# alonbebchuk/GNN-Pretraining

Hardware: AMD Instinct MI355X
Metric: pretrain graphs/sec (s4 multi-task) (higher is better)
Workload: dtype fp32; 1 GPU; s4 (NFM+LP+NC+GC+GP) pre-training step, 4 domains x 8 synthetic ENZYMES-shaped graphs per rank (input dims 7/4/37/21, hidden 256, 5 GIN layers), PCGrad + clip + AdamW; global_batch_graphs=32, parallelism=dp1, setup_steps=30, full=False, index_rng=reference, index_draws=native (csrc_host/hostdraw.cpp), cross_stream_sync=gates, ranks=1, devices_visible=1

## Files before the change

gnn_pretraining_amd/csrc/optim.hip:

```cpp
#include "gnnmp_internal.h"

namespace {

constexpr int MAXT = 8;
constexpr int CH = 32;
constexpr int GCH = 32;
constexpr int TB = 256;

struct MtArgs {
    const float* tg;
    int64_t stride;
    int T, K;
    int k0, k1;
    const int64_t* off;
    const int* len;
    const unsigned char* has;
    double* gram;
    double* gram_part;
    float* weights;
    int* flags;
    float* steps;
    int* metrics;
    int* block_metrics;
    int order[MAXT];
    int n_order;
    int last_task;
    int extra_task;
    float* final_grad;
    float* partial;
    float* normsq;
    float* params;
    float* exp_avg;
    float* exp_avg_sq;
    const float* lr;
    const float* wd;
    float beta1, beta2, eps, max_norm;
    const int* abort;
};

constexpr int MINP4 = 1024;
__device__ __forceinline__ int chunk_per4(int len4, int nch) { return max((len4 + nch - 1) / nch, MINP4); }
__device__ __forceinline__ int chunk_count(int len, int nch) {
    const int len4 = (len + 3) / 4;
    return len4 > 0 ? (len4 + chunk_per4(len4, nch) - 1) / chunk_per4(len4, nch) : 1;
}
__device__ __forceinline__ bool locate_chunk(const MtArgs& a, int k0, int k1, int nch, int b, int* k_out, int* j_out) {
    __shared__ int s_kj[2];
    if (threadIdx.x < 64) {
        const int lane = threadIdx.x;
        if (lane == 0) s_kj[0] = -1;
        int base = 0;
        for (int t0 = k0; t0 < k1; t0 += 64) {
            const int k = t0 + lane;
            const int cnt = k < k1 ? chunk_count(a.len[k], nch) : 0;
            int incl = cnt;
#pragma unroll
            for (int o = 1; o < 64; o <<= 1) {
                const int v = __shfl_up(incl, o, 64);
                if (lane >= o) incl += v;
            }
            const int excl = base + incl - cnt;
            if (cnt > 0 && b >= excl && b < excl + cnt) {
                s_kj[0] = k;
                s_kj[1] = b - excl;
            }
            base += __shfl(incl, 63, 64);
            if (base > b) break;
        }
    }
    __syncthreads();
    *k_out = s_kj[0];
    *j_out = s_kj[1];
    return s_kj[0] >= 0;
}

template <int NT>
__global__ __launch_bounds__(TB) void gram_kernel(const MtArgs a) {
    int k, j;
    if (!locate_chunk(a, a.k0, a.k1, GCH, blockIdx.x, &k, &j)) return;
    const int len = a.len[k], per = 4 * chunk_per4((len + 3) / 4, GCH);
    bool has[NT];
    int nh = 0;
#pragma unroll
    for (int t = 0; t < NT; ++t) {
        has[t] = t < a.T && a.has[k * MAXT + t];
        nh += has[t];
    }
    if (nh < 2) return;
    const int lo = j * per, hi = min(lo + per, (len + 3) / 4 * 4);
    double* out = a.gram_part + ((int64_t)k * GCH + j) * (MAXT * MAXT);
    constexpr int NP = NT * (NT + 1) / 2, NW = TB / 64, IT = 4;
    float acc[NP];
#pragma unroll
    for (int p = 0; p < NP; ++p) acc[p] = 0.f;
    const int64_t off = a.off[k];
    for (int i0 = lo + 4 * threadIdx.x; i0 < hi; i0 += IT * 4 * TB) {
        float4 g[IT][NT];
#pragma unroll
        for (int u = 0; u < IT; ++u) {
            const int i = i0 + u * 4 * TB;
#pragma unroll
            for (int t = 0; t < NT; ++t)
                g[u][t] = (has[t] && i < hi) ? *reinterpret_cast<const float4*>(a.tg + (int64_t)t * a.stride + off + i) : make_float4(0.f, 0.f, 0.f, 0.f);
        }
#pragma unroll
        for (int u = 0; u < IT; ++u) {
            int p = 0;
#pragma unroll
            for (int x = 0; x < NT; ++x)
#pragma unroll
                for (int y = x; y < NT; ++y, ++p) {
                    acc[p] += g[u][x].x * g[u][y].x;
                    acc[p] += g[u][x].y * g[u][y].y;
                    acc[p] += g[u][x].z * g[u][y].z;
                    acc[p] += g[u][x].w * g[u][y].w;
                }
        }
    }
    __shared__ double sh[NW][NP];
    const int lane = threadIdx.x % 64, wv = threadIdx.x / 64;
#pragma unroll
    for (int p = 0; p < NP; ++p) {
        float v = acc[p];
#pragma unroll
        for (int o = 32; o > 0; o >>= 1) v += __shfl_xor(v, o, 64);
        if (lane == 0) sh[wv][p] = (double)v;
    }
    __syncthreads();
    if (threadIdx.x < NP) {
        int x = 0, rem = threadIdx.x;
        while (rem >= NT - x) { rem -= NT - x; ++x; }
        const int y = x + rem;
        if (a.has[k * MAXT + x] && a.has[k * MAXT + y]) {
            double v = sh[0][threadIdx.x];
#pragma unroll
            for (int w = 1; w < NW; ++w) v += sh[w][threadIdx.x];
            out[x * MAXT + y] = v;
        }
    }
}

__global__ __launch_bounds__(64) void gram_finish_kernel(MtArgs a) {
    const int k = a.k0 + blockIdx.x, x = threadIdx.x / MAXT, y = threadIdx.x % MAXT;
    if (x >= a.T || y >= a.T || x > y) return;
    if (!a.has[k * MAXT + x] || !a.has[k * MAXT + y]) return;
    double s = 0.0;
    const int cnt = chunk_count(a.len[k], GCH);
    double v[GCH];
#pragma unroll
    for (int j = 0; j < GCH; ++j) v[j] = j < cnt ? a.gram_part[((int64_t)k * GCH + j) * (MAXT * MAXT) + x * MAXT + y] : 0.0;
#pragma unroll
    for (int j = 0; j < GCH; ++j) s += v[j];
    a.gram[((int64_t)k * MAXT + x) * MAXT + y] = s;
    a.gram[((int64_t)k * MAXT + y) * MAXT + x] = s;
}

__global__ __launch_bounds__(64) void solve_kernel(const MtArgs a) {
    __shared__ int s_conf[64], s_proj[64];
    int conf = 0, proj = 0;
    const int k = a.k0 + blockIdx.x * 64 + threadIdx.x;
    if (k < a.k1) {
        const unsigned char* has = a.has + k * MAXT;
        const double* G = a.gram + (int64_t)k * MAXT * MAXT;
        int flag = 0;
        float wout[MAXT];
#pragma unroll
        for (int i = 0; i < MAXT; ++i) wout[i] = 0.f;
        bool hp[MAXT];
        int nh = 0;
#pragma unroll
        for (int i = 0; i < MAXT; ++i) {
            hp[i] = i < a.n_order && has[a.order[i]];
            nh += hp[i];
        }
        if (nh > 1 || hp[0]) {
            double Gp[MAXT][MAXT];
#pragma unroll
            for (int i = 0; i < MAXT; ++i)
#pragma unroll
                for (int j = 0; j < MAXT; ++j) Gp[i][j] = (hp[i] && hp[j]) ? G[a.order[i] * MAXT + a.order[j]] : 0.0;
            double alpha[MAXT][MAXT];
#pragma unroll
            for (int i = 0; i < MAXT; ++i)
#pragma unroll
                for (int j = 0; j < MAXT; ++j) alpha[i][j] = i == j ? 1.0 : 0.0;
#pragma unroll
            for (int i = 1; i < MAXT; ++i) {
                if (!hp[i]) continue;
#pragma unroll
                for (int j = 0; j < i; ++j) {
                    if (!hp[j]) continue;
                    double ni = 0.0, dot = 0.0;
#pragma unroll
                    for (int p = 0; p <= i; ++p) {
                        double row = 0.0;
#pragma unroll
                        for (int q = 0; q <= i; ++q) row += alpha[i][q] * Gp[p][q];
                        ni += alpha[i][p] * row;
                        dot += alpha[i][p] * Gp[p][j];
                    }
                    const double nj = Gp[j][j];
                    if (ni <= 0.0 || nj <= 0.0) continue;
                    ++proj;
                    if (dot < 0.0) {
                        ++conf;
                        alpha[i][j] -= dot / nj;
                    }
                }
            }
#pragma unroll
            for (int i = 0; i < MAXT; ++i)
                if (hp[i]) {
#pragma unroll
                    for (int b = 0; b < MAXT; ++b) wout[b] += (float)(alpha[i][b] / nh);
                }
            flag = hp[0] ? 1 : 0;
        }
        float* w = a.weights + k * MAXT;
        for (int t = 0; t < MAXT; ++t) w[t] = 0.f;
        if (flag) {
#pragma unroll
            for (int i = 0; i < MAXT; ++i)
                if (i < a.n_order) w[a.order[i]] = wout[i];
        } else if (a.last_task >= 0 && has[a.last_task]) {
            w[a.last_task] = 1.f;
            flag = 1;
        }
        if (a.extra_task >= 0 && has[a.extra_task]) {
            w[a.extra_task] += 1.f;
            flag = 1;
        }
        a.flags[k] = flag;
        if (a.steps && !(a.abort && *a.abort)) a.steps[k] += (float)flag;
    }
    s_conf[threadIdx.x] = conf;
    s_proj[threadIdx.x] = proj;
    __syncthreads();
    for (int d = 32; d > 0; d >>= 1) {
        if (threadIdx.x < d) {
            s_conf[threadIdx.x] += s_conf[threadIdx.x + d];
            s_proj[threadIdx.x] += s_proj[threadIdx.x + d];
        }
        __syncthreads();
    }
    if (threadIdx.x == 0) {
        a.block_metrics[2 * (a.k0 + blockIdx.x)] = s_conf[0];
        a.block_metrics[2 * (a.k0 + blockIdx.x) + 1] = s_proj[0];
    }
    if (blockIdx.x == 0)
        for (int i = (int)gridDim.x + threadIdx.x; i < a.k1 - a.k0; i += 64) {
            a.block_metrics[2 * (a.k0 + i)] = 0;
            a.block_metrics[2 * (a.k0 + i) + 1] = 0;
        }
}

__global__ __launch_bounds__(TB) void combine_kernel(MtArgs a) {
    __shared__ float sh[TB / 64];
    int k, j;
    if (!locate_chunk(a, a.k0, a.k1, CH, blockIdx.x, &k, &j)) return;
    float ss = 0.f;
    if (a.flags[k]) {
        float w[MAXT];
        for (int t = 0; t < MAXT; ++t) w[t] = a.weights[k * MAXT + t];
        const int len4 = (a.len[k] + 3) / 4, per = chunk_per4(len4, CH);
        const int lo = j * per, hi = min(lo + per, len4);
        const int64_t off = a.off[k];
        for (int i = lo + threadIdx.x; i < hi; i += TB) {
            float4 g = make_float4(0.f, 0.f, 0.f, 0.f);
            for (int t = 0; t < a.T; ++t)
                if (w[t] != 0.f) {
                    const float4 v = *reinterpret_cast<const float4*>(a.tg + (int64_t)t * a.stride + off + 4 * (int64_t)i);
                    g = make_float4(fmaf(w[t], v.x, g.x), fmaf(w[t], v.y, g.y), fmaf(w[t], v.z, g.z), fmaf(w[t], v.w, g.w));
                }
            *reinterpret_cast<float4*>(a.final_grad + off + 4 * (int64_t)i) = g;
            ss = fmaf(g.x, g.x, ss); ss = fmaf(g.y, g.y, ss); ss = fmaf(g.z, g.z, ss); ss = fmaf(g.w, g.w, ss);
        }
    }
#pragma unroll
    for (int o = 32; o > 0; o >>= 1) ss += __shfl_xor(ss, o, 64);
    if (threadIdx.x % 64 == 0) sh[threadIdx.x / 64] = ss;
    __syncthreads();
    if (threadIdx.x == 0) {
        float s = sh[0];
        for (int w = 1; w < TB / 64; ++w) s += sh[w];
        a.partial[k * CH + j] = s;
    }
}

__global__ __launch_bounds__(TB) void foreign_kernel(MtArgs a) {
    __shared__ float sh[TB / 64];
    int k, j;
    if (!locate_chunk(a, a.k0, a.k1, CH, blockIdx.x, &k, &j)) return;
    const unsigned char* has = a.has + k * MAXT;
    int flag = a.n_order > 0 && has[a.order[0]] ? 1 : 0;
    if (!flag && a.last_task >= 0 && has[a.last_task]) flag = 1;
    if (a.extra_task >= 0 && has[a.extra_task]) flag = 1;
    if (j == 0 && threadIdx.x == 0) {
        a.flags[k] = flag;
        if (a.steps && !(a.abort && *a.abort)) a.steps[k] += (float)flag;
        a.block_metrics[2 * k] = 0;
        a.block_metrics[2 * k + 1] = 0;
    }
    float ss = 0.f;
    if (flag) {
        const int len4 = (a.len[k] + 3) / 4, per = chunk_per4(len4, CH);
        const int lo = j * per, hi = min(lo + per, len4);
        const int64_t off = a.off[k];
        for (int i = lo + threadIdx.x; i < hi; i += TB) {
            const float4 g = *reinterpret_cast<const float4*>(a.final_grad + off + 4 * (int64_t)i);
            ss = fmaf(g.x, g.x, ss); ss = fmaf(g.y, g.y, ss); ss = fmaf(g.z, g.z, ss); ss = fmaf(g.w, g.w, ss);
        }
    }
#pragma unroll
    for (int o = 32; o > 0; o >>= 1) ss += __shfl_xor(ss, o, 64);
    if (threadIdx.x % 64 == 0) sh[threadIdx.x / 64] = ss;
    __syncthreads();
    if (threadIdx.x == 0) {
        float s2 = sh[0];
        for (int w = 1; w < TB / 64; ++w) s2 += sh[w];
        a.partial[k * CH + j] = s2;
    }
}

__global__ __launch_bounds__(TB) void norm_kernel(MtArgs a) {
    __shared__ double sh[TB];
    __shared__ int shc[TB], shp[TB];
    double s = 0.0;
    for (int k = threadIdx.x; k < a.K; k += TB) {
        const int cnt = chunk_count(a.len[k], CH);
        const float4* row = reinterpret_cast<const float4*>(a.partial + (int64_t)k * CH);
        float4 v[CH / 4];
#pragma unroll
        for (int q = 0; q < CH / 4; ++q) v[q] = 4 * q < cnt ? row[q] : make_float4(0.f, 0.f, 0.f, 0.f);
#pragma unroll
        for (int q = 0; q < CH / 4; ++q) {
            if (4 * q + 0 < cnt) s += (double)v[q].x;
            if (4 * q + 1 < cnt) s += (double)v[q].y;
            if (4 * q + 2 < cnt) s += (double)v[q].z;
            if (4 * q + 3 < cnt) s += (double)v[q].w;
        }
    }
    int c = 0, pr = 0;
    for (int b = threadIdx.x; b < a.K; b += TB) {
        c += a.block_metrics[2 * b];
        pr += a.block_metrics[2 * b + 1];
    }
    sh[threadIdx.x] = s;
    shc[threadIdx.x] = c;
    shp[threadIdx.x] = pr;
    __syncthreads();
    for (int d = TB / 2; d > 0; d >>= 1) {
        if (threadIdx.x < d) {
            sh[threadIdx.x] += sh[threadIdx.x + d];
            shc[threadIdx.x] += shc[threadIdx.x + d];
            shp[threadIdx.x] += shp[threadIdx.x + d];
        }
        __syncthreads();
    }
    if (threadIdx.x == 0) {
        a.normsq[0] = (float)sh[0];
        a.metrics[0] = shc[0];
        a.metrics[1] = shp[0];
    }
}

__global__ __launch_bounds__(TB) void adamw_kernel(MtArgs a) {
    int k, j;
    if (!locate_chunk(a, 0, a.K, CH, blockIdx.x, &k, &j)) return;
    if (!a.flags[k]) return;
    if (a.abort && *a.abort) return;
    float coef = 1.f;
    if (a.max_norm > 0.f) coef = fminf(1.f, a.max_norm / (sqrtf(a.normsq[0]) + 1e-6f));
    const float lr = a.lr[k], wd = a.wd[k], step = a.steps[k];
    const float bc1 = 1.f - powf(a.beta1, step), bc2 = 1.f - powf(a.beta2, step);
    const float step_size = lr / bc1, bc2s = sqrtf(bc2);
    const int len4 = (a.len[k] + 3) / 4, per = chunk_per4(len4, CH);
    const int lo = j * per, hi = min(lo + per, len4);
    const int64_t off = a.off[k];
    auto one = [&](float g, float p, float m0, float v0, float* mo, float* vo) -> float {
        g *= coef;
        p *= (1.f - lr * wd);
        const float m = m0 + (g - m0) * (1.f - a.beta1);
        const float v = v0 * a.beta2 + g * g * (1.f - a.beta2);
        *mo = m;
        *vo = v;
        return p - step_size * (m / (sqrtf(v) / bc2s + a.eps));
    };
    for (int i = lo + threadIdx.x; i < hi; i += TB) {
        const int64_t o = off + 4 * (int64_t)i;
        const float4 g = *reinterpret_cast<const float4*>(a.final_grad + o), p = *reinterpret_cast<const float4*>(a.params + o);
        const float4 m0 = *reinterpret_cast<const float4*>(a.exp_avg + o), v0 = *reinterpret_cast<const float4*>(a.exp_avg_sq + o);
        float4 m, v, q;
        q.x = one(g.x, p.x, m0.x, v0.x, &m.x, &v.x);
        q.y = one(g.y, p.y, m0.y, v0.y, &m.y, &v.y);
        q.z = one(g.z, p.z, m0.z, v0.z, &m.z, &v.z);
        q.w = one(g.w, p.w, m0.w, v0.w, &m.w, &v.w);
        *reinterpret_cast<float4*>(a.exp_avg + o) = m;
        *reinterpret_cast<float4*>(a.exp_avg_sq + o) = v;
        *reinterpret_cast<float4*>(a.params + o) = q;
    }
}

}

extern "C" size_t gmp_mt_workspace_bytes(int num_tensors) {
    const size_t K = num_tensors > 0 ? num_tensors : 0;
    return K * MAXT * MAXT * sizeof(double) * (1 + GCH) + K * MAXT * sizeof(float) + K * sizeof(int) + K * CH * sizeof(float) +
           (K + 2) * 2 * sizeof(int) + 1024;
}

extern "C" int gmp_mt_pcgrad_clip_adamw_ex(const float* task_grads, int64_t task_stride, int num_tasks, int num_tensors,
                                           const int64_t* tensor_off, const int32_t* tensor_len, const uint8_t* has,
                                           const int32_t* order_host, int n_order, int last_task, int extra_task,
                                           float* params, float* exp_avg, float* exp_avg_sq, float* steps,
                                           const float* lr, const float* wd, float beta1, float beta2, float eps,
                                           float max_norm, float* final_grad, float* normsq_out, int32_t* metrics_out,
                                           int32_t* flags_out, void* ws, size_t ws_bytes, int apply_update,
                                           int k_begin, int k_end, int phases, const int32_t* abort_flag, gmp_stream_t stream) {
    if (k_begin < 0 || k_end > num_tensors || k_begin > k_end || !(phases & 7))
        return gmp::fail(GMP_ERR_ARG, "mt_pcgrad: tensors [%d, %d) of %d, phases %d", k_begin, k_end, num_tensors, phases);
    if (num_tasks < 1 || num_tasks > MAXT || num_tensors < 1 || n_order < 1 || n_order > num_tasks)
        return gmp::fail(GMP_ERR_ARG, "mt_pcgrad: tasks=%d tensors=%d n_order=%d", num_tasks, num_tensors, n_order);
    if (!task_grads || !tensor_off || !tensor_len || !has || !order_host || !final_grad || !normsq_out || !metrics_out || !flags_out || !ws)
        return gmp::fail(GMP_ERR_ARG, "mt_pcgrad: null pointer");
    if (apply_update && (!params || !exp_avg || !exp_avg_sq || !steps || !lr || !wd)) return gmp::fail(GMP_ERR_ARG, "mt_pcgrad: optimizer state");
    if (ws_bytes < gmp_mt_workspace_bytes(num_tensors)) return gmp::fail(GMP_ERR_WORKSPACE, "mt_pcgrad: workspace");
    if (last_task >= num_tasks || extra_task >= num_tasks) return gmp::fail(GMP_ERR_ARG, "mt_pcgrad: task index");
    MtArgs a{};
    a.tg = task_grads; a.stride = task_stride; a.T = num_tasks; a.K = num_tensors; a.off = tensor_off; a.len = tensor_len;
    a.k0 = k_begin; a.k1 = k_end;
    a.has = has;
    char* w = (char*)ws;
    a.gram = (double*)w; w += (size_t)num_tensors * MAXT * MAXT * sizeof(double);
    a.gram_part = (double*)w; w += (size_t)num_tensors * GCH * MAXT * MAXT * sizeof(double);
    a.weights = (float*)w; w += (size_t)num_tensors * MAXT * sizeof(float);
    a.partial = (float*)w; w += (size_t)num_tensors * CH * sizeof(float);
    a.block_metrics = (int*)w;
    a.flags = flags_out; a.steps = steps; a.metrics = metrics_out;
    for (int i = 0; i < n_order; ++i) {
        if (order_host[i] < 0 || order_host[i] >= num_tasks) return gmp::fail(GMP_ERR_ARG, "mt_pcgrad: order[%d]=%d", i, order_host[i]);
        a.order[i] = order_host[i];
    }
    a.n_order = n_order; a.last_task = last_task; a.extra_task = extra_task;
    a.final_grad = final_grad; a.normsq = normsq_out; a.params = params; a.exp_avg = exp_avg; a.exp_avg_sq = exp_avg_sq;
    a.lr = lr; a.wd = wd; a.beta1 = beta1; a.beta2 = beta2; a.eps = eps; a.max_norm = max_norm;
    a.abort = abort_flag;
    hipStream_t st = (hipStream_t)stream;
    const int nk = k_end - k_begin;
    auto nblk = [&](int n) { return (unsigned)(task_stride / (4 * MINP4) + 2 * (int64_t)n + 1); };
    if ((phases & 1) && nk > 0) {
        if (n_order > 1) {
            switch (num_tasks) {
                case 2: hipLaunchKernelGGL(gram_kernel<2>, dim3(nblk(nk)), dim3(TB), 0, st, a); break;
                case 3: hipLaunchKernelGGL(gram_kernel<3>, dim3(nblk(nk)), dim3(TB), 0, st, a); break;
                case 4: hipLaunchKernelGGL(gram_kernel<4>, dim3(nblk(nk)), dim3(TB), 0, st, a); break;
                case 5: hipLaunchKernelGGL(gram_kernel<5>, dim3(nblk(nk)), dim3(TB), 0, st, a); break;
                case 6: hipLaunchKernelGGL(gram_kernel<6>, dim3(nblk(nk)), dim3(TB), 0, st, a); break;
                default: hipLaunchKernelGGL(gram_kernel<MAXT>, dim3(nblk(nk)), dim3(TB), 0, st, a); break;
            }
            hipLaunchKernelGGL(gram_finish_kernel, dim3(nk), dim3(64), 0, st, a);
        }
        hipLaunchKernelGGL(solve_kernel, dim3((nk + 63) / 64), dim3(64), 0, st, a);
        hipLaunchKernelGGL(combine_kernel, dim3(nblk(nk)), dim3(TB), 0, st, a);
    }
    if ((phases & 4) && nk > 0) hipLaunchKernelGGL(foreign_kernel, dim3(nblk(nk)), dim3(TB), 0, st, a);
    if (phases & 2) {
        hipLaunchKernelGGL(norm_kernel, dim3(1), dim3(TB), 0, st, a);
        if (apply_update) hipLaunchKernelGGL(adamw_kernel, dim3(nblk(num_tensors)), dim3(TB), 0, st, a);
    }
    return gmp::check_launch("mt_pcgrad_clip_adamw kernels");
}

extern "C" int gmp_mt_pcgrad_clip_adamw(const float* task_grads, int64_t task_stride, int num_tasks, int num_tensors,
                                        const int64_t* tensor_off, const int32_t* tensor_len, const uint8_t* has,
                                        const int32_t* order_host, int n_order, int last_task, int extra_task,
                                        float* params, float* exp_avg, float* exp_avg_sq, float* steps,
                                        const float* lr, const float* wd, float beta1, float beta2, float eps,
                                        float max_norm, float* final_grad, float* normsq_out, int32_t* metrics_out,
                                        int32_t* flags_out, void* ws, size_t ws_bytes, int apply_update,
                                        gmp_stream_t stream) {
    return gmp_mt_pcgrad_clip_adamw_ex(task_grads, task_stride, num_tasks, num_tensors, tensor_off, tensor_len, has, order_host, n_order,
                                       last_task, extra_task, params, exp_avg, exp_avg_sq, steps, lr, wd, beta1, beta2, eps, max_norm,
                                       final_grad, normsq_out, metrics_out, flags_out, ws, ws_bytes, apply_update, 0, num_tensors, 3, nullptr, stream);
}
```

gnn_pretraining_amd/engine.py:

```python
from __future__ import annotations

import ctypes as C
import os
import random
from typing import Dict, List, Optional, Sequence, Tuple

import numpy as np
import torch
from torch import Tensor

from . import _lib as L
from .constants import DOMAIN_DIMENSIONS, GRAPH_PROPERTY_DIM
from .graph import Batch
from .models.gnn import DROPOUT_RATE, GNN_HIDDEN_DIM, GNN_NUM_LAYERS
from .models.pretrain_model import PretrainableGNN, draw_mask_indices
from .pretrain.augmentations import _augment_one
from .pretrain.control import DEFAULT_LR, DEFAULT_WEIGHT_DECAY, TASK_SPECIFIC_LR
from .pretrain.tasks import sample_negative_edges

H = GNN_HIDDEN_DIM
NT, NN, TN = 0, 1, 2
MAXT = 8
SEG_CSR_MAX_ROWS, SEG_CSR_MAX_EDGES = 8192, 24576

# ... 278 lines not shown
        return bool(self.use_gates and self.native and os.environ.get("GMP_UPLOAD_ON_AUX", "1") != "0")

    @property
    def parts_beside_backward(self) -> bool:
        return bool(self._parts_ok and self.native)

    def _flatten_parameters(self) -> None:
        m, dev = self.model, self.device
        named = dict(m.named_parameters())
        enc = [m.input_encoders[d] for d in self.domains]
        order: List[Tuple[str, Tensor]] = []
        for d, e in zip(self.domains, enc):
            order.append((f"input_encoders.{d}.linear.weight", e.linear.weight))
        for key in ("linear.bias", "batch_norm.weight", "batch_norm.bias"):
            for d in self.domains:
                order.append((f"input_encoders.{d}.{key}", named[f"input_encoders.{d}.{key}"]))
        seen = {n for n, _ in order}
        for n, p in named.items():
            if n not in seen:
                order.append((n, p))
        al4 = lambda v: (v + 3) // 4 * 4
        self.off: Dict[str, int] = {}
        o = 0
        for n, p in order:
            self.off[n] = o
            o += al4(p.numel())
        self.P = o
        self.P_shared = min(self.off[n] for n, _ in order if n.startswith("heads.")) if any(n.startswith("heads.") for n, _ in order) else o
        self.flat = torch.zeros(self.P, device=dev)
        for n, p in order:
            o = self.off[n]
            self.flat[o:o + p.numel()].copy_(p.data.reshape(-1))
            p.data = self.flat[o:o + p.numel()].view_as(p)
        self.names = [n for n, _ in order]
        self.numel = {n: p.numel() for n, p in order}
        self.enc_rm = torch.zeros(self.D, H, device=dev)
        self.enc_rv = torch.ones(self.D, H, device=dev)
        for i, e in enumerate(enc):
            self.enc_rm[i].copy_(e.batch_norm.running_mean)
            self.enc_rv[i].copy_(e.batch_norm.running_var)
            e.batch_norm.running_mean.data = self.enc_rm[i]
            e.batch_norm.running_var.data = self.enc_rv[i]
        self.exp_avg = torch.zeros(self.P, device=dev)
        self.exp_avg_sq = torch.zeros(self.P, device=dev)

    def _build_tables(self) -> None:
        dev, T = self.device, self.T
        K = len(self.names)
        self.K = K
        self.t_off = torch.tensor([self.off[n] for n in self.names], dtype=torch.int64, device=dev)
        self.t_len = torch.tensor([self.numel[n] for n in self.names], dtype=torch.int32, device=dev)
        has = np.zeros((K, MAXT), dtype=np.uint8)
        lr = np.zeros(K, dtype=np.float32)
        for k, n in enumerate(self.names):
            lr[k] = DEFAULT_LR
            if n.startswith("input_encoders."):
                for t, task in enumerate(self.tasks):
                    has[k, t] = task != "node_feat_mask"
            elif n == "mask_token":
                for t, task in enumerate(self.tasks):
                    has[k, t] = task == "node_feat_mask"
            elif n.startswith("gnn_backbone."):
                has[k, :T] = 1
            elif n.startswith("heads."):
                for t, task in enumerate(self.tasks):
                    if f"heads.{task}" in n:
                        has[k, t] = 1
                        lr[k] = TASK_SPECIFIC_LR[task]
        self.has_static = has
        self.has = torch.from_numpy(has.copy()).to(dev)
        self.lr = torch.from_numpy(lr).to(dev)
        self.wd = torch.full((K,), DEFAULT_WEIGHT_DECAY, dtype=torch.float32, device=dev)
        self.steps = torch.zeros(K, dtype=torch.float32, device=dev)
        self.name_index = {n: k for k, n in enumerate(self.names)}

    def _alloc(self) -> None:
        dev, R = self.device, self.max_rows
        f = lambda *shape: torch.empty(*shape, device=dev)
        self.task_grads = torch.zeros(self.T, self.P, device=dev)
        self.final_grad = torch.zeros(self.P, device=dev)
        self.normsq = torch.zeros(1, device=dev)
        self.metrics = torch.zeros(2, dtype=torch.int32, device=dev)
        self.flags = torch.zeros(self.K, dtype=torch.int32, device=dev)
        self.mt_ws = torch.empty(self.lib.gmp_mt_workspace_bytes(self.K), dtype=torch.uint8, device=dev)
        Lr = GNN_NUM_LAYERS
        self.z0 = f(R, H)
        self.h = [f(R, H) for _ in range(Lr + 1)]
        self.a = [f(R, H) for _ in range(Lr)]
        self.z1 = [f(R, 2 * H) for _ in range(Lr)]
        self.r1 = [f(R, 2 * H) for _ in range(Lr)]
        self.z2 = [f(R, H) for _ in range(Lr)]
        self.S_MAX = 64
        self.stat = {k: f(Lr, self.S_MAX, c) for k, c in (("m1", 2 * H), ("s1", 2 * H), ("m2", H), ("s2", H))}
        self.enc_mean, self.enc_rstd = f(self.S_MAX, H), f(self.S_MAX, H)
        self.gA, self.gB = f(R, H), f(R, H)
        self.ga = f(R, H)
        self.gW = f(R, 2 * H)
        self.gW2 = f(R, 2 * H)
        self.gB2, self.gW3 = f(R, H), f(R, 2 * H)
        self.gu_l, self.gz1_l = [f(R, H) for _ in range(Lr)], [f(R, 2 * H) for _ in range(Lr)]
        self.rowdot = f(Lr * R)
        self.gemm_ws = torch.empty(48 << 20, dtype=torch.uint8, device=dev)
        from . import streams as ST
        self.aux_stream, *extra = ST.concurrent_streams(dev, 3)
        self.sync_flags = torch.zeros(64, dtype=torch.int32, device=dev)
        self._epoch = 0
        self.use_gates = bool(ST.last_report.get("calibrated") and ST.last_report.get("own_queue") == 3
                              and os.environ.get("GMP_STEP_GATES", "1") != "0")
        self._parts_ok = (self.use_gates and os.environ.get("GMP_DP_OVERLAP", "1") != "0" and os.environ.get("GMP_OPT_OVERLAP", "0") == "1")
        self.comm_stream = extra[1]
        bins = [[0.0, extra[0]], [0.0, extra[1]], [0.0, self.aux_stream], [0.0, None]]
        self.task_streams = [None] * self.T
        for ti in sorted(range(self.T), key=lambda i: -HEAD_CHAIN_US.get(self.tasks[i], 100.0)):
            b = min(bins, key=lambda x: x[0])
            b[0] += HEAD_CHAIN_US.get(self.tasks[ti], 100.0)
            self.task_streams[ti] = b[1]
        self.task_gemm_ws = [torch.empty(24 << 20, dtype=torch.uint8, device=dev) for _ in range(self.T)]
        self.task_loss_ws = [torch.empty(self.lib.gmp_loss_workspace_bytes(R * H), dtype=torch.uint8, device=dev) for _ in range(self.T)]
        self._cur_gemm_ws = self.gemm_ws
        self.bn_ws = torch.empty(12 * self.lib.gmp_bn_workspace_bytes(R, 2 * H, self.S_MAX, R), dtype=torch.uint8, device=dev)
        self.csr_ws = torch.empty(self.lib.gmp_csr_build_workspace_bytes(R, self.max_edges), dtype=torch.uint8, device=dev)
        i32 = lambda n: torch.empty(n, dtype=torch.int32, device=dev)
        self.csr = [i32(R + 1), i32(self.max_edges), i32(self.max_edges), i32(R + 1), i32(self.max_edges), i32(self.max_edges)]
        self.csr_status = i32(1)
        self.lp_csr_status = i32(1)
        self.lp_csr_ws = torch.empty(self.lib.gmp_csr_build_workspace_bytes(R, self.max_edges), dtype=torch.uint8, device=dev)
        self.lp_csr = [i32(R + 1), i32(self.max_edges), i32(self.max_edges), i32(R + 1), i32(self.max_edges), i32(self.max_edges)]
        self.loss_sums = torch.zeros(MAXT, device=dev)
        self.loss_ws = torch.empty(self.lib.gmp_loss_workspace_bytes(R * H), dtype=torch.uint8, device=dev)
        self.KMAX = self.max_edges
        self.hd = {k: f(n, c) for k, (n, c) in {
            "nfm_in": (R, H), "nfm_y1": (R, H), "nfm_d1": (R, H), "nfm_y2": (R, H), "nfm_tgt": (R, H), "nfm_g": (R, H), "nfm_g1": (R, H), "nfm_gin": (R, H),
            "lp_feat": (self.KMAX, 3 * H), "lp_y1": (self.KMAX, H), "lp_d1": (self.KMAX, H), "lp_gy1": (self.KMAX, H),
            "lp_gfeat": (self.KMAX, 3 * H), "lp_ghs": (self.KMAX, H), "lp_ghd": (self.KMAX, H),
            "nc_in": (2 * R, H), "nc_y1": (2 * R, H), "nc_d1": (2 * R, H), "nc_z": (2 * R, 128), "nc_gz": (2 * R, 128), "nc_g1": (2 * R, H), "nc_gin": (2 * R, H),
            "gc_mean": (1024, H), "gc_max": (1024, H), "gc_in": (1024, 2 * H), "gc_y1": (1024, H), "gc_d1": (1024, H), "gc_z": (1024, 128),
            "gc_gz": (1024, 128), "gc_g1": (1024, H), "gc_gin": (1024, 2 * H), "gc_gmean": (1024, H), "gc_gmax": (1024, H),
            "da_in": (1024, H), "da_y1": (1024, DA_HIDDEN), "da_d1": (1024, DA_HIDDEN), "da_logits": (1024, 8), "da_glogits": (1024, 8),
            "da_g1": (1024, DA_HIDDEN), "da_gin": (1024, H),
            "gp_in": (1024, H), "gp_y1": (1024, 2 * H), "gp_d1": (1024, 2 * H), "gp_y2": (1024, 16), "gp_g2": (1024, 16), "gp_g1": (1024, 2 * H), "gp_gin": (1024, H),
        }.items()}
        self.lp_y2, self.lp_p, self.lp_gp, self.lp_gy2 = f(2 * self.KMAX), f(2 * self.KMAX), f(self.KMAX), f(2 * self.KMAX)
        self.gp_y2 = f(1024, GRAPH_PROPERTY_DIM)
        self.gp_g2 = f(1024, GRAPH_PROPERTY_DIM)
        self.ntx_ws = [torch.empty(self.lib.gmp_nt_xent_grouped_workspace_bytes(self.D, 512, 128), dtype=torch.uint8, device=dev) for _ in range(2 * self.D)]
        self.i32_cap, self.i64_cap = 4 * R + 8 * self.S_MAX + 65536 + 2 * self.max_edges, 4 * self.max_edges + 8 * R
        self.STAGES = 4
        self.stage = [{"pin32": torch.empty(self.i32_cap, dtype=torch.int32).pin_memory(),
                       "pin64": torch.empty(self.i64_cap, dtype=torch.int64).pin_memory(),
                       "pinf": torch.empty(64 + self.KMAX, dtype=torch.float32).pin_memory(),
                       "event": None} for _ in range(self.STAGES)]
        self._up_sets = [(torch.empty(self.i32_cap, dtype=torch.int32, device=dev), torch.empty(self.i64_cap, dtype=torch.int64, device=dev),
                          torch.zeros(64, device=dev), f(self.KMAX)) for _ in range(2)]
        self.dev32, self.dev64, self.scal, self.lp_lab = self._up_sets[0]

    def draw(self, inp: StepInputs, gen: torch.Generator) -> Dict[str, object]:
        if self.rng_mode == "vectorized":
            return self._draw_vectorized(inp, gen)
        if self.rng_mode == "device":
            return self.collect_draws(inp, self.enqueue_draws(inp))
        art: Dict[str, object] = {}
        host = {d: inp.host[d] for d in self.domains}
        H = hostdraw()
        if H is not None and hasattr(H, "draw_step"):
            if self._neg_native is None:
                self._neg_native = H.PyRandom()
                self._neg_native.setstate(torch.tensor(self.neg_rng.getstate()[1], dtype=torch.long))
# ... 1501 lines not shown
```

gnn_pretraining_amd/finetune/engine.py:

```python
from __future__ import annotations

import ctypes as C
import os as _os_mod
from typing import Dict, List, NamedTuple, Optional, Tuple

import torch
from torch import Tensor

from .. import _lib as L, operators as OP, ops
from ..graph import SparseFeatures
from ..models.finetune_model import LR_BACKBONE, LR_FINETUNE, FinetuneGNN
from ..models.gnn import DROPOUT_RATE, GNN_HIDDEN_DIM, GNN_NUM_LAYERS

H = GNN_HIDDEN_DIM
NT, NN, TN = 0, 1, 2
ADAMW_WEIGHT_DECAY = 0.01


def _i32(xs):
    return (C.c_int32 * len(xs))(*[int(v) for v in xs])


def _i64(xs):
    return (C.c_int64 * len(xs))(*[int(v) for v in xs])


class NodeClassificationEngine:
    def __init__(self, model: FinetuneGNN, x: Tensor, edge_index: Tensor, device, seed: int = 0) -> None:
        self.model, self.device, self.lib = model, torch.device(device), L.lib()
        self.seed, self.step_count, self.dropout_p = seed, 0, DROPOUT_RATE
        dev = self.device
        self.N, self.d_in = int(x.size(0)), int(x.size(1))
        self.dpad = (self.d_in + 31) // 32 * 32
        self.sparse = isinstance(x, SparseFeatures)
        if self.sparse:
            self.x, self.xs = None, x.to(dev)
            self.x_csc = self.xs.csc()
            self.sp_wt = torch.empty(self.lib.gmp_sparse_linear_workspace_bytes(self.d_in, H), dtype=torch.uint8, device=dev)
            self.sp_status = torch.zeros(1, dtype=torch.int32, device=dev)
            self.colsum_ws = torch.empty(max(self.lib.gmp_colsum_workspace_bytes(self.N, H), 16), dtype=torch.uint8, device=dev)
        else:
            self.x = torch.zeros(self.N, self.dpad, device=dev)
            self.x[:, :self.d_in] = x.to(dev)
        self.csr = ops.csr_build(edge_index.to(dev).contiguous(), self.N)
        head = model.classification_head
        self.classes = int(head.mlp[0].weight.size(0)) if hasattr(head, "mlp") else 0
        self._flatten()
        f = lambda *s: torch.empty(*s, device=dev)
        N, Lr = self.N, GNN_NUM_LAYERS
        self.z0, self.h = f(N, H), [f(N, H) for _ in range(Lr + 1)]
        self.a, self.z1, self.r1, self.z2 = [f(N, H) for _ in range(Lr)], [f(N, 2 * H) for _ in range(Lr)], [f(N, 2 * H) for _ in range(Lr)], [f(N, H) for _ in range(Lr)]
        self.stat = {k: f(Lr, c) for k, c in (("m1", 2 * H), ("s1", 2 * H), ("m2", H), ("s2", H))}
        self.enc_mean, self.enc_rstd = f(H), f(H)
        self.logits, self.gA, self.gB, self.ga, self.gW, self.gW2 = f(N, self.classes), f(N, H), f(N, H), f(N, H), f(N, 2 * H), f(N, 2 * H)
        self.gu_l, self.gz1_l = [f(N, H) for _ in range(Lr + 1)], [f(N, 2 * H) for _ in range(Lr)]
        self.rowdot = f(Lr, N)
        if dev.type == "cuda":
            from .. import streams as ST
            self.side = ST.concurrent_streams(dev, 1)[0]
            own_queue = not ST.share_queue(torch.cuda.current_stream(dev).cuda_stream, self.side.cuda_stream)
            self._gates_ok = own_queue and _os_mod.environ.get("GMP_FINETUNE_GATES", "1") != "0"
        else:
            self.side, self._gates_ok, own_queue = None, False, False
        self.sync_flags = torch.zeros(64, dtype=torch.int32, device=dev)
        self._epoch = 0
        self.side_ws = torch.empty(32 << 20, dtype=torch.uint8, device=dev)
        self.seed_word = torch.zeros(1, dtype=torch.int64, device=dev)
        import os as _os
        self.use_graph = dev.type == "cuda" and _os.environ.get("GMP_FINETUNE_GRAPH", "0") == "1"
        self.fork_wgrads = _os.environ.get("GMP_FINETUNE_FORK", "0" if (self.use_graph or not own_queue) else "1") == "1"
        self._graph, self._graph_key, self._graph_step, self._graph_seen = None, None, -1, None
        self.seg_ptr = torch.tensor([0, N], dtype=torch.int32, device=dev)
        self.bn_ws = torch.empty(self.lib.gmp_bn_workspace_bytes(N, 2 * H, 1, N), dtype=torch.uint8, device=dev)
        self.bn_sync = (torch.zeros(self.lib.gmp_bn_sync_bytes(2 * H, 1) // 4, dtype=torch.int32, device=dev)
                        if _os.environ.get("GMP_BN_SLABS", "1") != "0" else None)
        self.gemm_ws = torch.empty(32 << 20, dtype=torch.uint8, device=dev)
        self.loss_ws = torch.empty(self.lib.gmp_loss_workspace_bytes(N * H), dtype=torch.uint8, device=dev)
        self.loss_sum, self.g_scale = torch.zeros(1, device=dev), torch.ones(1, device=dev)
        self.mt_ws = torch.empty(self.lib.gmp_mt_workspace_bytes(self.K), dtype=torch.uint8, device=dev)
        self.normsq, self.metrics, self.flags = torch.zeros(1, device=dev), torch.zeros(2, dtype=torch.int32, device=dev), torch.zeros(self.K, dtype=torch.int32, device=dev)
        self._train_idx: Optional[Tensor] = None
        self._bn_calls = 0
        self._fold_ch = [H] + [2 * H, H] * GNN_NUM_LAYERS
        self._fold_off = [2 * sum(self._fold_ch[:i]) for i in range(len(self._fold_ch))]
        self._fold_table = torch.empty(2 * sum(self._fold_ch), device=dev)
        self._infer_loss: Optional[Tuple[Tensor, int]] = None
        self._fwd_gen, self._embed_gen = 0, -1

    def _flatten(self) -> None:
        m, dev = self.model, self.device
        named = [(n, p) for n, p in m.named_parameters()]
        al4 = lambda v: (v + 3) // 4 * 4
        self.off: Dict[str, int] = {}
        self.numel: Dict[str, int] = {}
        o = 0
        for n, p in named:
            cnt = H * self.dpad if n == "input_encoder.linear.weight" else p.numel()
            self.off[n], self.numel[n] = o, cnt
            o += al4(cnt)
        self.P = o
        self.flat = torch.zeros(self.P, device=dev)
        for n, p in named:
            a = self.off[n]
            if n == "input_encoder.linear.weight":
                view = self.flat[a:a + H * self.dpad].view(H, self.dpad)
                view[:, :self.d_in].copy_(p.data)
                p.data = view[:, :self.d_in]
            else:
                self.flat[a:a + p.numel()].copy_(p.data.reshape(-1))
                p.data = self.flat[a:a + p.numel()].view_as(p)
        self.names = [n for n, _ in named]
        self.K = len(self.names)
        self.grad = torch.zeros(1, self.P, device=dev)
        self.final_grad = torch.zeros(self.P, device=dev)
        self.exp_avg, self.exp_avg_sq = torch.zeros(self.P, device=dev), torch.zeros(self.P, device=dev)
        self.t_off = torch.tensor([self.off[n] for n in self.names], dtype=torch.int64, device=dev)
        self.t_len = torch.tensor([self.numel[n] for n in self.names], dtype=torch.int32, device=dev)
        trainable = {n: p.requires_grad for n, p in named}
        has = torch.zeros(self.K, 8, dtype=torch.uint8)
        lr = torch.zeros(self.K)
        for k, n in enumerate(self.names):
            has[k, 0] = 1 if trainable[n] else 0
            lr[k] = LR_BACKBONE if n.startswith("gnn_backbone.") else LR_FINETUNE
        self.has, self.lr = has.to(dev), lr.to(dev)
        self.wd = torch.full((self.K,), ADAMW_WEIGHT_DECAY, device=dev)
        self.steps = torch.zeros(self.K, device=dev)

    def _P(self, n: str) -> int:
        return self.flat.data_ptr() + 4 * self.off[n]

    def _G(self, n: str) -> int:
        return self.off[n]

    def _chk(self, rc: int, what: str) -> None:
        if rc:
            L.check(rc, what)

    def _cfg(self, relu: bool, dropout: bool, site: int) -> L.BnConfig:
        p = self.dropout_p if (dropout and self.model.training) else 0.0
        base = self.seed * 1000003
        sync = (self.bn_sync.data_ptr(), self.bn_sync.numel()) if self.bn_sync is not None else (None, 0)
        if self._seed_dev:
            return L.BnConfig(int(self.model.training), int(relu), 1e-5, 0.1, p, base & (2 ** 64 - 1), site + self._site_base, self._seed_dev, *sync)
        return L.BnConfig(int(self.model.training), int(relu), 1e-5, 0.1, p, (base + self.step_count) & (2 ** 64 - 1), site + self._site_base, None, *sync)

    _seed_dev = None
    _site_base = 0

    def _gemm(self, st, mode, A, B, bias, Cc, M, N, K, lda, ldb, ldc, ws: Optional[Tensor] = None):
        self._chk(self.lib.gmp_gemm_f32(mode, A, B, bias, Cc, M, N, K, lda, ldb, ldc, 1.0, 0, 0, None if ws is None else ws.data_ptr(),
                                        0 if ws is None else ws.numel(), st), "gemm")

    def _wgrad(self, st, G, X, w_name: str, b_name: str, M_tn: int, N_out: int, ldx: int, ws: Optional[Tensor] = None):
        g, ws = self.grad.data_ptr(), (self.gemm_ws if ws is None else ws)
        self._chk(self.lib.gmp_gemm_f32_grouped(TN, G, X, None, g, 1, _i32([0, self.N]), None, None, _i64([self._G(w_name)]), g, _i64([self._G(b_name)]),
                                                M_tn, N_out, 0, M_tn, ldx, N_out, 1.0, 0, 0, ws.data_ptr(), ws.numel(), st), "wgrad")

    def forward(self) -> Tensor:
        self._backbone_forward()
        self._gemm(torch.cuda.current_stream(self.device).cuda_stream, NT, self.h[GNN_NUM_LAYERS].data_ptr(), self._P("classification_head.mlp.0.weight"),
                   self._P("classification_head.mlp.0.bias"), self.logits.data_ptr(), self.N, self.classes, H, H, H, self.classes)
        if self.model.training:
# ... 561 lines not shown
```

Before: 24230 graphs/s.

## Fuse PCGrad gram reduce, solve, and norm into fewer kernels via last-block tickets

Uses per-tensor atomic tickets so that the last gram chunk block of each tensor reduces the partial Gram entries and runs the PCGrad solve inline, removing the gram_finish and solve launches. Single-owner tensors get their weights computed directly in gram or combine. The norm reduction is folded into the AdamW kernel, with each live block recomputing the global norm, which removes another launch. The cost is redundant norm work per block, extra atomics, and a zero-initialised workspace needed for the tickets. A GMP_MT_FUSED=0 setting keeps the old path.

```diff
diff --git a/gnn_pretraining_amd/csrc/optim.hip b/gnn_pretraining_amd/csrc/optim.hip
--- a/gnn_pretraining_amd/csrc/optim.hip
+++ b/gnn_pretraining_amd/csrc/optim.hip
@@ -1,3 +1,5 @@
+#include <stdlib.h>
+
 #include "gnnmp_internal.h"
 
 namespace {
@@ -22,6 +24,7 @@
     float* steps;
     int* metrics;
     int* block_metrics;
+    int* tickets;
     int order[MAXT];
     int n_order;
     int last_task;
@@ -74,7 +77,120 @@
     return s_kj[0] >= 0;
 }
 
-template <int NT>
+template <int NPOS>
+__device__ __forceinline__ void solve_tensor(const MtArgs& a, int k, const double* G, int* conf_out, int* proj_out) {
+    int conf = 0, proj = 0;
+    const unsigned char* has = a.has + k * MAXT;
+    int flag = 0;
+    float wout[NPOS];
+#pragma unroll
+    for (int i = 0; i < NPOS; ++i) wout[i] = 0.f;
+    bool hp[NPOS];
+    int nh = 0;
+#pragma unroll
+    for (int i = 0; i < NPOS; ++i) {
+        hp[i] = i < a.n_order && has[a.order[i]];
+        nh += hp[i];
+    }
+    if (nh > 1 || hp[0]) {
+        double Gp[NPOS][NPOS];
+#pragma unroll
+        for (int i = 0; i < NPOS; ++i)
+#pragma unroll
+            for (int j = 0; j < NPOS; ++j) Gp[i][j] = (hp[i] && hp[j]) ? G[a.order[i] * MAXT + a.order[j]] : 0.0;
+        double alpha[NPOS][NPOS];
+#pragma unroll
+        for (int i = 0; i < NPOS; ++i)
+#pragma unroll
+            for (int j = 0; j < NPOS; ++j) alpha[i][j] = i == j ? 1.0 : 0.0;
+#pragma unroll
+        for (int i = 1; i < NPOS; ++i) {
+            if (!hp[i]) continue;
+#pragma unroll
+            for (int j = 0; j < i; ++j) {
+                if (!hp[j]) continue;
+                double ni = 0.0, dot = 0.0;
+#pragma unroll
+                for (int p = 0; p <= i; ++p) {
+                    double row = 0.0;
+#pragma unroll
+                    for (int q = 0; q <= i; ++q) row += alpha[i][q] * Gp[p][q];
+                    ni += alpha[i][p] * row;
+                    dot += alpha[i][p] * Gp[p][j];
+                }
+                const double nj = Gp[j][j];
+                if (ni <= 0.0 || nj <= 0.0) continue;
+                ++proj;
+                if (dot < 0.0) {
+                    ++conf;
+                    alpha[i][j] -= dot / nj;
+                }
+            }
+        }
+#pragma unroll
+        for (int i = 0; i < NPOS; ++i)
+            if (hp[i]) {
+#pragma unroll
+                for (int b = 0; b < NPOS; ++b) wout[b] += (float)(alpha[i][b] / nh);
+            }
+        flag = hp[0] ? 1 : 0;
+    }
+    float* w = a.weights + k * MAXT;
+    for (int t = 0; t < MAXT; ++t) w[t] = 0.f;
+    if (flag) {
+#pragma unroll
+        for (int i = 0; i < NPOS; ++i)
+            if (i < a.n_order) w[a.order[i]] = wout[i];
+    } else if (a.last_task >= 0 && has[a.last_task]) {
+        w[a.last_task] = 1.f;
+        flag = 1;
+    }
+    if (a.extra_task >= 0 && has[a.extra_task]) {
+        w[a.extra_task] += 1.f;
+        flag = 1;
+    }
+    a.flags[k] = flag;
+    if (a.steps && !(a.abort && *a.abort)) a.steps[k] += (float)flag;
+    *conf_out = conf;
+    *proj_out = proj;
+}
+
+struct OneOwner {
+    int t_main, t_extra, flag;
+    __device__ __forceinline__ float weight(int t) const { return (t == t_main ? 1.f : 0.f) + (t == t_extra ? 1.f : 0.f); }
+};
+__device__ __forceinline__ OneOwner solve_one_owner(const MtArgs& a, int k) {
+    const unsigned char* has = a.has + k * MAXT;
+    OneOwner r;
+    r.t_main = has[a.order[0]] ? a.order[0] : (a.last_task >= 0 && has[a.last_task]) ? a.last_task : -1;
+    r.t_extra = (a.extra_task >= 0 && has[a.extra_task]) ? a.extra_task : -1;
+    r.flag = (r.t_main >= 0 || r.t_extra >= 0) ? 1 : 0;
+    return r;
+}
+__device__ __forceinline__ void publish_one_owner(const MtArgs& a, int k, const OneOwner& r) {
+    for (int t = 0; t < MAXT; ++t) a.weights[k * MAXT + t] = r.weight(t);
+    a.flags[k] = r.flag;
+    if (a.steps && !(a.abort && *a.abort)) a.steps[k] += (float)r.flag;
+    a.block_metrics[2 * k] = 0;
+    a.block_metrics[2 * k + 1] = 0;
+}
+
+template <bool COHERENT>
+__device__ __forceinline__ double gram_entry(const MtArgs& a, int k, int x, int y) {
+    double s = 0.0;
+    const int cnt = chunk_count(a.len[k], GCH);
+    double v[GCH];
+#pragma unroll
+    for (int j = 0; j < GCH; ++j) {
+        const double* p = a.gram_part + ((int64_t)k * GCH + j) * (MAXT * MAXT) + x * MAXT + y;
+        v[j] = j >= cnt ? 0.0 : COHERENT ? __hip_atomic_load(p, __ATOMIC_RELAXED, __HIP_MEMORY_SCOPE_AGENT) : *p;
+    }
+#pragma unroll
+    for (int j = 0; j < GCH; ++j) s += v[j];
+    return s;
+}
+
+template <int NT, bool FUSED>
 __global__ __launch_bounds__(TB) void gram_kernel(const MtArgs a) {
     int k, j;
     if (!locate_chunk(a, a.k0, a.k1, GCH, blockIdx.x, &k, &j)) return;
@@ -86,7 +202,10 @@
         has[t] = t < a.T && a.has[k * MAXT + t];
         nh += has[t];
     }
-    if (nh < 2) return;
+    if (nh < 2) {
+        if (FUSED && j == 0 && threadIdx.x == 0) publish_one_owner(a, k, solve_one_owner(a, k));
+        return;
+    }
     const int lo = j * per, hi = min(lo + per, (len + 3) / 4 * 4);
     double* out = a.gram_part + ((int64_t)k * GCH + j) * (MAXT * MAXT);
     constexpr int NP = NT * (NT + 1) / 2, NW = TB / 64, IT = 4;
@@ -135,8 +254,39 @@
             double v = sh[0][threadIdx.x];
 #pragma unroll
             for (int w = 1; w < NW; ++w) v += sh[w][threadIdx.x];
-            out[x * MAXT + y] = v;
-        }
+            if (FUSED) __hip_atomic_store(out + x * MAXT + y, v, __ATOMIC_RELAXED, __HIP_MEMORY_SCOPE_AGENT);
+            else out[x * MAXT + y] = v;
+        }
+    }
+    if (!FUSED) return;
+    __shared__ int s_last;
+    __shared__ double s_gram[MAXT * MAXT];
+    asm volatile("s_waitcnt vmcnt(0)" ::: "memory");
+    __syncthreads();
+    if (threadIdx.x == 0) {
+        const int cnt = chunk_count(len, GCH);
+        const int mine = __hip_atomic_fetch_add(a.tickets + k, 1, __ATOMIC_RELAXED, __HIP_MEMORY_SCOPE_AGENT);
+        s_last = mine == cnt - 1;
+        if (mine == cnt - 1) __hip_atomic_store(a.tickets + k, 0, __ATOMIC_RELAXED, __HIP_MEMORY_SCOPE_AGENT);
+    }
+    __syncthreads();
+    if (!s_last) return;
+    if (threadIdx.x < MAXT * MAXT) {
+        const int x = threadIdx.x / MAXT, y = threadIdx.x % MAXT;
+        if (x < a.T && y < a.T && x <= y && a.has[k * MAXT + x] && a.has[k * MAXT + y]) {
+            const double s = gram_entry<true>(a, k, x, y);
+            a.gram[((int64_t)k * MAXT + x) * MAXT + y] = s;
+            a.gram[((int64_t)k * MAXT + y) * MAXT + x] = s;
+            s_gram[x * MAXT + y] = s;
+            s_gram[y * MAXT + x] = s;
+        }
+    }
+    __syncthreads();
+    if (threadIdx.x == 0) {
+        int conf, proj;
+        solve_tensor<NT>(a, k, s_gram, &conf, &proj);
+        a.block_metrics[2 * k] = conf;
+        a.block_metrics[2 * k + 1] = proj;
     }
 }
 
@@ -144,13 +294,7 @@
     const int k = a.k0 + blockIdx.x, x = threadIdx.x / MAXT, y = threadIdx.x % MAXT;
     if (x >= a.T || y >= a.T || x > y) return;
     if (!a.has[k * MAXT + x] || !a.has[k * MAXT + y]) return;
-    double s = 0.0;
-    const int cnt = chunk_count(a.len[k], GCH);
-    double v[GCH];
-#pragma unroll
-    for (int j = 0; j < GCH; ++j) v[j] = j < cnt ? a.gram_part[((int64_t)k * GCH + j) * (MAXT * MAXT) + x * MAXT + y] : 0.0;
-#pragma unroll
-    for (int j = 0; j < GCH; ++j) s += v[j];
+    const double s = gram_entry<false>(a, k, x, y);
     a.gram[((int64_t)k * MAXT + x) * MAXT + y] = s;
     a.gram[((int64_t)k * MAXT + y) * MAXT + x] = s;
 }
@@ -159,80 +303,7 @@
     __shared__ int s_conf[64], s_proj[64];
     int conf = 0, proj = 0;
     const int k = a.k0 + blockIdx.x * 64 + threadIdx.x;
-    if (k < a.k1) {
-        const unsigned char* has = a.has + k * MAXT;
-        const double* G = a.gram + (int64_t)k * MAXT * MAXT;
-        int flag = 0;
-        float wout[MAXT];
-#pragma unroll
-        for (int i = 0; i < MAXT; ++i) wout[i] = 0.f;
-        bool hp[MAXT];
-        int nh = 0;
-#pragma unroll
-        for (int i = 0; i < MAXT; ++i) {
-            hp[i] = i < a.n_order && has[a.order[i]];
-            nh += hp[i];
-        }
-        if (nh > 1 || hp[0]) {
-            double Gp[MAXT][MAXT];
-#pragma unroll
-            for (int i = 0; i < MAXT; ++i)
-#pragma unroll
-                for (int j = 0; j < MAXT; ++j) Gp[i][j] = (hp[i] && hp[j]) ? G[a.order[i] * MAXT + a.order[j]] : 0.0;
-            double alpha[MAXT][MAXT];
-#pragma unroll
-            for (int i = 0; i < MAXT; ++i)
-#pragma unroll
-                for (int j = 0; j < MAXT; ++j) alpha[i][j] = i == j ? 1.0 : 0.0;
-#pragma unroll
-            for (int i = 1; i < MAXT; ++i) {
-                if (!hp[i]) continue;
-#pragma unroll
-                for (int j = 0; j < i; ++j) {
-                    if (!hp[j]) continue;
-                    double ni = 0.0, dot = 0.0;
-#pragma unroll
-                    for (int p = 0; p <= i; ++p) {
-                        double row = 0.0;
-#pragma unroll
-                        for (int q = 0; q <= i; ++q) row += alpha[i][q] * Gp[p][q];
-                        ni += alpha[i][p] * row;
-                        dot += alpha[i][p] * Gp[p][j];
-                    }
-                    const double nj = Gp[j][j];
-                    if (ni <= 0.0 || nj <= 0.0) continue;
-                    ++proj;
-                    if (dot < 0.0) {
-                        ++conf;
-                        alpha[i][j] -= dot / nj;
-                    }
-                }
-            }
-#pragma unroll
-            for (int i = 0; i < MAXT; ++i)
-                if (hp[i]) {
-#pragma unroll
-                    for (int b = 0; b < MAXT; ++b) wout[b] += (float)(alpha[i][b] / nh);
-                }
-            flag = hp[0] ? 1 : 0;
-        }
-        float* w = a.weights + k * MAXT;
-        for (int t = 0; t < MAXT; ++t) w[t] = 0.f;
-        if (flag) {
-#pragma unroll
-            for (int i = 0; i < MAXT; ++i)
-                if (i < a.n_order) w[a.order[i]] = wout[i];
-        } else if (a.last_task >= 0 && has[a.last_task]) {
-            w[a.last_task] = 1.f;
-            flag = 1;
-        }
-        if (a.extra_task >= 0 && has[a.extra_task]) {
-            w[a.extra_task] += 1.f;
-            flag = 1;
-        }
-        a.flags[k] = flag;
-        if (a.steps && !(a.abort && *a.abort)) a.steps[k] += (float)flag;
-    }
+    if (k < a.k1) solve_tensor<MAXT>(a, k, a.gram + (int64_t)k * MAXT * MAXT, &conf, &proj);
     s_conf[threadIdx.x] = conf;
     s_proj[threadIdx.x] = proj;
     __syncthreads();
@@ -254,14 +325,20 @@
         }
 }
 
+template <bool SOLVE>
 __global__ __launch_bounds__(TB) void combine_kernel(MtArgs a) {
     __shared__ float sh[TB / 64];
     int k, j;
     if (!locate_chunk(a, a.k0, a.k1, CH, blockIdx.x, &k, &j)) return;
     float ss = 0.f;
-    if (a.flags[k]) {
+    OneOwner own{};
+    if (SOLVE) {
+        own = solve_one_owner(a, k);
+        if (j == 0 && threadIdx.x == 0) publish_one_owner(a, k, own);
+    }
+    if (SOLVE ? own.flag : a.flags[k]) {
         float w[MAXT];
-        for (int t = 0; t < MAXT; ++t) w[t] = a.weights[k * MAXT + t];
+        for (int t = 0; t < MAXT; ++t) w[t] = SOLVE ? own.weight(t) : a.weights[k * MAXT + t];
         const int len4 = (a.len[k] + 3) / 4, per = chunk_per4(len4, CH);
         const int lo = j * per, hi = min(lo + per, len4);
         const int64_t off = a.off[k];
@@ -322,7 +399,7 @@
     }
 }
 
-__global__ __launch_bounds__(TB) void norm_kernel(MtArgs a) {
+__device__ __forceinline__ double total_normsq(const MtArgs& a, bool counts, int* conf_out, int* proj_out) {
     __shared__ double sh[TB];
     __shared__ int shc[TB], shp[TB];
     double s = 0.0;
@@ -341,10 +418,11 @@
         }
     }
     int c = 0, pr = 0;
-    for (int b = threadIdx.x; b < a.K; b += TB) {
-        c += a.block_metrics[2 * b];
-        pr += a.block_metrics[2 * b + 1];
-    }
+    if (counts)
+        for (int b = threadIdx.x; b < a.K; b += TB) {
+            c += a.block_metrics[2 * b];
+            pr += a.block_metrics[2 * b + 1];
+        }
     sh[threadIdx.x] = s;
     shc[threadIdx.x] = c;
     shp[threadIdx.x] = pr;
@@ -357,20 +435,42 @@
         }
         __syncthreads();
     }
+    *conf_out = shc[0];
+    *proj_out = shp[0];
+    return sh[0];
+}
+
+__global__ __launch_bounds__(TB) void norm_kernel(MtArgs a) {
+    int conf, proj;
+    const double s = total_normsq(a, true, &conf, &proj);
     if (threadIdx.x == 0) {
-        a.normsq[0] = (float)sh[0];
-        a.metrics[0] = shc[0];
-        a.metrics[1] = shp[0];
-    }
-}
-
+        a.normsq[0] = (float)s;
+        a.metrics[0] = conf;
+        a.metrics[1] = proj;
+    }
+}
+
+template <bool NORM>
 __global__ __launch_bounds__(TB) void adamw_kernel(MtArgs a) {
     int k, j;
-    if (!locate_chunk(a, 0, a.K, CH, blockIdx.x, &k, &j)) return;
-    if (!a.flags[k]) return;
-    if (a.abort && *a.abort) return;
+    const bool mine = locate_chunk(a, 0, a.K, CH, blockIdx.x, &k, &j);
+    const bool live = mine && a.flags[k] && !(a.abort && *a.abort);
+    float normsq = 0.f;
+    if (NORM) {
+        if (blockIdx.x == 0 || (live && a.max_norm > 0.f)) {
+            int conf, proj;
+            normsq = (float)total_normsq(a, blockIdx.x == 0, &conf, &proj);
+            if (blockIdx.x == 0 && threadIdx.x == 0) {
+                a.normsq[0] = normsq;
+                a.metrics[0] = conf;
+                a.metrics[1] = proj;
+            }
+        }
+    }
+    if (!live) return;
+    if (!NORM) normsq = a.normsq[0];
     float coef = 1.f;
-    if (a.max_norm > 0.f) coef = fminf(1.f, a.max_norm / (sqrtf(a.normsq[0]) + 1e-6f));
+    if (a.max_norm > 0.f) coef = fminf(1.f, a.max_norm / (sqrtf(normsq) + 1e-6f));
     const float lr = a.lr[k], wd = a.wd[k], step = a.steps[k];
     const float bc1 = 1.f - powf(a.beta1, step), bc2 = 1.f - powf(a.beta2, step);
     const float step_size = lr / bc1, bc2s = sqrtf(bc2);
@@ -406,7 +506,7 @@
 extern "C" size_t gmp_mt_workspace_bytes(int num_tensors) {
     const size_t K = num_tensors > 0 ? num_tensors : 0;
     return K * MAXT * MAXT * sizeof(double) * (1 + GCH) + K * MAXT * sizeof(float) + K * sizeof(int) + K * CH * sizeof(float) +
-           (K + 2) * 2 * sizeof(int) + 1024;
+           (K + 2) * 2 * sizeof(int) + 1024 + K * sizeof(int);
 }
 
 extern "C" int gmp_mt_pcgrad_clip_adamw_ex(const float* task_grads, int64_t task_stride, int num_tasks, int num_tensors,
@@ -436,6 +536,7 @@
     a.weights = (float*)w; w += (size_t)num_tensors * MAXT * sizeof(float);
     a.partial = (float*)w; w += (size_t)num_tensors * CH * sizeof(float);
     a.block_metrics = (int*)w;
+    a.tickets = (int*)((char*)ws + gmp_mt_workspace_bytes(num_tensors)) - num_tensors;
     a.flags = flags_out; a.steps = steps; a.metrics = metrics_out;
     for (int i = 0; i < n_order; ++i) {
         if (order_host[i] < 0 || order_host[i] >= num_tasks) return gmp::fail(GMP_ERR_ARG, "mt_pcgrad: order[%d]=%d", i, order_host[i]);
@@ -447,26 +548,37 @@
     a.abort = abort_flag;
     hipStream_t st = (hipStream_t)stream;
     const int nk = k_end - k_begin;
+    const char* env = getenv("GMP_MT_FUSED");
+    const bool fused = !(env && atoi(env) == 0);
     auto nblk = [&](int n) { return (unsigned)(task_stride / (4 * MINP4) + 2 * (int64_t)n + 1); };
     if ((phases & 1) && nk > 0) {
         if (n_order > 1) {
+#define GMP_GRAM(NT)                                                                              \
+    if (fused) hipLaunchKernelGGL((gram_kernel<NT, true>), dim3(nblk(nk)), dim3(TB), 0, st, a);    \
+    else hipLaunchKernelGGL((gram_kernel<NT, false>), dim3(nblk(nk)), dim3(TB), 0, st, a)
             switch (num_tasks) {
-                case 2: hipLaunchKernelGGL(gram_kernel<2>, dim3(nblk(nk)), dim3(TB), 0, st, a); break;
-                case 3: hipLaunchKernelGGL(gram_kernel<3>, dim3(nblk(nk)), dim3(TB), 0, st, a); break;
-                case 4: hipLaunchKernelGGL(gram_kernel<4>, dim3(nblk(nk)), dim3(TB), 0, st, a); break;
-                case 5: hipLaunchKernelGGL(gram_kernel<5>, dim3(nblk(nk)), dim3(TB), 0, st, a); break;
-                case 6: hipLaunchKernelGGL(gram_kernel<6>, dim3(nblk(nk)), dim3(TB), 0, st, a); break;
-                default: hipLaunchKernelGGL(gram_kernel<MAXT>, dim3(nblk(nk)), dim3(TB), 0, st, a); break;
+                case 2: GMP_GRAM(2); break;
+                case 3: GMP_GRAM(3); break;
+                case 4: GMP_GRAM(4); break;
+                case 5: GMP_GRAM(5); break;
+                case 6: GMP_GRAM(6); break;
+                default: GMP_GRAM(MAXT); break;
             }
-            hipLaunchKernelGGL(gram_finish_kernel, dim3(nk), dim3(64), 0, st, a);
-        }
-        hipLaunchKernelGGL(solve_kernel, dim3((nk + 63) / 64), dim3(64), 0, st, a);
-        hipLaunchKernelGGL(combine_kernel, dim3(nblk(nk)), dim3(TB), 0, st, a);
+#undef GMP_GRAM
+            if (!fused) hipLaunchKernelGGL(gram_finish_kernel, dim3(nk), dim3(64), 0, st, a);
+        }
+        if (!fused) hipLaunchKernelGGL(solve_kernel, dim3((nk + 63) / 64), dim3(64), 0, st, a);
+        if (fused && n_order == 1) hipLaunchKernelGGL(combine_kernel<true>, dim3(nblk(nk)), dim3(TB), 0, st, a);
+        else hipLaunchKernelGGL(combine_kernel<false>, dim3(nblk(nk)), dim3(TB), 0, st, a);
     }
     if ((phases & 4) && nk > 0) hipLaunchKernelGGL(foreign_kernel, dim3(nblk(nk)), dim3(TB), 0, st, a);
     if (phases & 2) {
-        hipLaunchKernelGGL(norm_kernel, dim3(1), dim3(TB), 0, st, a);
-        if (apply_update) hipLaunchKernelGGL(adamw_kernel, dim3(nblk(num_tensors)), dim3(TB), 0, st, a);
+        if (fused && apply_update) {
+            hipLaunchKernelGGL(adamw_kernel<true>, dim3(nblk(num_tensors)), dim3(TB), 0, st, a);
+        } else {
+            hipLaunchKernelGGL(norm_kernel, dim3(1), dim3(TB), 0, st, a);
+            if (apply_update) hipLaunchKernelGGL(adamw_kernel<false>, dim3(nblk(num_tensors)), dim3(TB), 0, st, a);
+        }
     }
     return gmp::check_launch("mt_pcgrad_clip_adamw kernels");
 }
diff --git a/gnn_pretraining_amd/engine.py b/gnn_pretraining_amd/engine.py
--- a/gnn_pretraining_amd/engine.py
+++ b/gnn_pretraining_amd/engine.py
@@ -384,7 +384,7 @@
         self.normsq = torch.zeros(1, device=dev)
         self.metrics = torch.zeros(2, dtype=torch.int32, device=dev)
         self.flags = torch.zeros(self.K, dtype=torch.int32, device=dev)
-        self.mt_ws = torch.empty(self.lib.gmp_mt_workspace_bytes(self.K), dtype=torch.uint8, device=dev)
+        self.mt_ws = torch.zeros(self.lib.gmp_mt_workspace_bytes(self.K), dtype=torch.uint8, device=dev)
         Lr = GNN_NUM_LAYERS
         self.z0 = f(R, H)
         self.h = [f(R, H) for _ in range(Lr + 1)]
diff --git a/gnn_pretraining_amd/finetune/engine.py b/gnn_pretraining_amd/finetune/engine.py
--- a/gnn_pretraining_amd/finetune/engine.py
+++ b/gnn_pretraining_amd/finetune/engine.py
@@ -77,7 +77,7 @@
         self.gemm_ws = torch.empty(32 << 20, dtype=torch.uint8, device=dev)
         self.loss_ws = torch.empty(self.lib.gmp_loss_workspace_bytes(N * H), dtype=torch.uint8, device=dev)
         self.loss_sum, self.g_scale = torch.zeros(1, device=dev), torch.ones(1, device=dev)
-        self.mt_ws = torch.empty(self.lib.gmp_mt_workspace_bytes(self.K), dtype=torch.uint8, device=dev)
+        self.mt_ws = torch.zeros(self.lib.gmp_mt_workspace_bytes(self.K), dtype=torch.uint8, device=dev)
         self.normsq, self.metrics, self.flags = torch.zeros(1, device=dev), torch.zeros(2, dtype=torch.int32, device=dev), torch.zeros(self.K, dtype=torch.int32, device=dev)
         self._train_idx: Optional[Tensor] = None
         self._bn_calls = 0
```

Measured after the change: 24430 graphs/s (median of 6 runs). No clear change (+0.8%).
